# VIPL-Audio-Visual-Speech-Understanding/SBL_For_Multilingual_Lip_Reading

Hardware: AMD Instinct MI355X
Metric: lip-clips/sec fwd+bwd (29x88x88) (higher is better)
Workload: dtype f32 (exact 3-way bf16 split, 6 bf16 MFMA products per fp32 product, fp32 accumulate); 1 GPU; full SBL 6+6 (Conv3d stem + ResNet-18 + encoder + SBL decoder) fwd+loss+bwd (BASELINE config 3); matmul_precision=bf16x6, per_gpu_batch=32, global_batch=32, clip=29x88x88, parallelism=dp1, dropout=True, bn=train, issue=graph, hipgraph=True, decoder_streams=2, conv_weight_pack=cached (re-packed when weights change), decoder_schedule=teacher-forced runs batched, coin_patterns=8

## Files before the change

### include/sbl_hip.h

```cpp
#ifndef SBL_HIP_H
#define SBL_HIP_H
#include <stdint.h>
#ifdef __cplusplus
extern "C" {
#endif

#define SBL_ERR_INVALID (-22)
#define SBL_ABI_VERSION 1

typedef void* sbl_stream_t;

const char* sbl_last_error(void);
int sbl_abi_version(void);

int sbl_profile_begin(uint64_t* stamps, int capacity);
int sbl_profile_end(void);
int sbl_profile_used(void);
int sbl_profile_last_slot(void);
int sbl_profile_last_kernel(void);

int sbl_set_matmul_precision(int terms);
int sbl_get_matmul_precision(void);
int sbl_set_tuning(int knob, int value);

// ... 48 lines not shown
int sbl_bn_bwd_apply(const float* dy, const float* y, const float* x, const float* mean, const float* invstd,
                     const float* gamma, const double* sums, float* dx, float* dres, float* dgamma, float* dbeta,
                     long rows, int C, int relu, int accumulate, sbl_stream_t stream);

int sbl_conv_weight_pack(const float* w_oihw, float* w_ohwi, float* w_dgrad , int Cout,
                         int Cin, int KH, int KW, double* zero , int nzero, sbl_stream_t stream);
int sbl_conv_wgrad_unpack(const float* dw_ohwi, float* dw_oihw, int Cout, int Cin, int KH, int KW, int accumulate,
                          sbl_stream_t stream);
int sbl_conv2d_fwd(const float* x, const float* w_ohwi, float* y, double* stats, int stats_zeroed, int NIMG, int H, int W, int Cin,
                   int Cout, int KH, int KW, int stride, int pad, void* ws, long ws_bytes, sbl_stream_t stream);
int sbl_conv2d_dgrad(const float* dy, const float* w_dgrad, float* dx, int NIMG, int H, int W, int Cin, int Cout,
                     int KH, int KW, int stride, int pad, void* ws, long ws_bytes, sbl_stream_t stream);
int sbl_conv2d_dgrad_bnstats(const float* dy, const float* w_dgrad, float* dx, int NIMG, int H, int W, int Cin, int Cout,
                             int KH, int KW, int stride, int pad, void* ws, long ws_bytes, const float* act,
                             const float* pre, const float* mean, const float* invstd, double* sums,
                             int sums_zeroed ,
                             sbl_stream_t stream);
int sbl_conv2d_dgrad_fused(const float* dy, const float* w_dgrad, float* dx, int NIMG, int H, int W, int Cin, int Cout,
                           int KH, int KW, int stride, int pad, void* ws, long ws_bytes, const float* addend,
                           const float* act, const float* pre, const float* mean, const float* invstd, const float* pre2,
                           const float* mean2, const float* invstd2, double* sums, int sums_zeroed, sbl_stream_t stream);
int sbl_conv1x1s2_dgrad_compact(const float* dy, const float* w_dgrad, float* dx_compact, int NIMG, int H, int W, int Cin,
                                int Cout, void* ws, long ws_bytes, sbl_stream_t stream);
int sbl_conv2d_wgrad(const float* x, const float* dy, float* dw_ohwi, int NIMG, int H, int W, int Cin, int Cout,
                     int KH, int KW, int stride, int pad, int dw_zeroed, sbl_stream_t stream);
int sbl_avgpool_fwd(const float* x, float* y, int NIMG, int HW, int C, sbl_stream_t stream);
int sbl_avgpool_bwd(const float* dy, float* dx, int NIMG, int HW, int C, sbl_stream_t stream);

int sbl_dropout(const float* x, float* y, long n, float p, const uint64_t* seed, uint64_t offset,
                sbl_stream_t stream);
int sbl_seed_bump(uint64_t* seed, sbl_stream_t stream);

int sbl_add_layernorm_fwd(const float* x, const float* res, const float* gamma, const float* beta, float* y,
                          float* mean, float* rstd, int M, int D, float eps, float drop_p, const uint64_t* seed,
                          uint64_t offset, sbl_stream_t stream);
int sbl_add_layernorm2_fusion_fwd(const float* x0, const float* x1, const float* res0, const float* res1, const float* gamma0,
// ... 161 lines not shown
```

### sbl_for_multilingual_lip_reading_amd/csrc/conv.hip

```cpp
#include "mfma_gemm.h"
#include "conv_patch.h"
#include "conv_patch_wgrad.h"

SblRouting g_sbl_route = {2, 30};
extern "C" int sbl_set_tuning(int knob, int value) {
    SBL_REQUIRE(knob == 5 || knob == 9, "sbl_set_tuning: no knob %d; the two that remain are 5 (patch-resident 3x3 / stride-1 forward / input gradient: 2 on, "
                "0 the per-tap gather kernels) and 9 (smallest map in pixels that takes the patch-resident weight gradient, 0 = never)", knob);
    if (knob == 5) {
        SBL_REQUIRE(value == 0 || value == 2, "sbl_set_tuning: knob 5 takes 2 (patch-resident kernels) or 0 (per-tap gather kernels), not %d", value);
        g_sbl_route.conv_patch = value;
    } else {
        SBL_REQUIRE(value >= 0, "sbl_set_tuning: negative value");
        g_sbl_route.conv_patch_wgrad = value;
    }
    return 0;
}

static int check_conv(const char* who, int NIMG, int H, int W, int Cin, int Cout, int KH, int KW, int stride, int pad) {
    SBL_REQUIRE(NIMG > 0 && H > 0 && W > 0, "%s: bad image dims %d %d %d", who, NIMG, H, W);
    SBL_REQUIRE(Cin % 16 == 0 && Cout % 16 == 0 && Cin >= 16 && Cout >= 16, "%s: Cin=%d Cout=%d must be multiples of 16", who, Cin, Cout);
    SBL_REQUIRE((KH == 3 && KW == 3 && pad == 1) || (KH == 1 && KW == 1 && pad == 0), "%s: only 3x3/pad1 and 1x1/pad0 (got %dx%d pad %d)", who, KH, KW, pad);
    SBL_REQUIRE(stride == 1 || stride == 2, "%s: stride %d", who, stride);
    SBL_REQUIRE(sbl_fits_u32((long)NIMG * H * W * (long)(Cin > Cout ? Cin : Cout)), "%s: tensor spans more than 2 GiB (buffer descriptor range)", who);
    SBL_REQUIRE((long)NIMG * H * W < (1L << 24) && Cin < (1 << 16) && Cout < (1 << 16), "%s: more than 2^24 pixels (24-bit index arithmetic in the gathers)", who);
// ... 28 lines not shown
static const RowMap kRowsDirect{0, 0, 0, 0, 0, 0, 0};
static inline RowMap rows_pm(int NIMG, int HW) { return RowMap{2, NIMG, HW, 0, 0, 0, 0}; }

struct DgradFuse {
    const float* addend;
    int add_class00;
    const float* y;
    const float* x;
    const float* mean;
    const float* inv;
    const float* x2;
    const float* mean2;
    const float* inv2;
    double* sums;
    int sums_zeroed;
};

static EpiStore<0, false> epi_plain(float* C, int N, const RowMap& r) {
    return {C, (long)N, nullptr, 0, nullptr, nullptr, 0, r.cmap, r.ca, r.cb, r.cH, r.cW, r.cph, r.cpw};
}
static EpiStore<0, true> epi_stats(float* C, int N, double* stats, const RowMap& r) {
    return {C, (long)N, nullptr, 0, stats, nullptr, 0, r.cmap, r.ca, r.cb, r.cH, r.cW, r.cph, r.cpw};
}
template <bool SUMS>
static EpiStore<0, SUMS, true> epi_fused(float* C, int N, const DgradFuse& f, const float* add, long add_ld, const RowMap& r) {
    const DgradFuse b = SUMS ? f : DgradFuse{};
    return {C, (long)N, nullptr, 0, b.sums, nullptr, 0, r.cmap, r.ca, r.cb, r.cH, r.cW, r.cph, r.cpw,
            b.y, b.x, b.mean, b.inv, b.x2, b.mean2, b.inv2, add, add_ld};
}
template <class F>
static auto with_fwd_epi(float* y, int N, double* stats, const RowMap& r, F&& fn) {
    if (stats) return fn(epi_stats(y, N, stats, r));
    return fn(epi_plain(y, N, r));
}
template <class F>
static auto with_dgrad_epi(float* dx, int N, const DgradFuse& f, F&& fn) {
    if (f.sums) return fn([&](const RowMap& r, const float* add, long add_ld) { return epi_fused<true>(dx, N, f, add, add_ld, r); });
    if (f.addend) return fn([&](const RowMap& r, const float* add, long add_ld) { return epi_fused<false>(dx, N, f, add, add_ld, r); });
    return fn([&](const RowMap& r, const float*, long) { return epi_plain(dx, N, r); });
}

template <class AL, class BL, class EPI, int BM, int BN>
// ... 26 lines not shown
}

extern "C" int sbl_conv2d_fwd(const float* x, const float* w, float* y, double* stats, int stats_zeroed, int NIMG, int H, int W,
                              int Cin, int Cout, int KH, int KW, int stride, int pad, void* ws, long ws_bytes, sbl_stream_t stream) {
    hipStream_t s = (hipStream_t)stream;
    if (int e = check_conv("sbl_conv2d_fwd", NIMG, H, W, Cin, Cout, KH, KW, stride, pad)) return e;
    SBL_REQUIRE(x && w && y && sbl_aligned16(x) && sbl_aligned16(w), "sbl_conv2d_fwd: null/unaligned pointer");
    const int Ho = out_dim(H, KH, stride, pad), Wo = out_dim(W, KW, stride, pad);
    const int M = NIMG * Ho * Wo, N = Cout, K = KH * KW * Cin;
    ConvGeom g{NIMG, Ho, Wo, H, W, Cin, KH, KW, stride, pad, 0, 0, 0, 0, {0, 0, 0, 0}, {0, 0, 0, 0}};
    sbl_geom_finish(g);
    if (stats && !stats_zeroed) SBL_HIP(hipMemsetAsync(stats, 0, sizeof(double) * 2 * Cout, s));
    SBL_REQUIRE(!ws || (sbl_aligned16(ws) && ws_bytes >= (long)sizeof(int) * kConvWsCounters), "sbl_conv2d_fwd: workspace unaligned or < 16 KiB");
    if (KH == 3 && stride == 1) {
        bool done;
        const PatchEpi pe{y, stats, nullptr, nullptr, nullptr, nullptr, nullptr, nullptr, nullptr, nullptr};
        if (stats) done = sbl_launch_conv_patch<false, 1>(x, w, pe, NIMG, H, W, Cin, Cout, SBL_KID_CONV_FWD, s);
        else done = sbl_launch_conv_patch<false, 0>(x, w, pe, NIMG, H, W, Cin, Cout, SBL_KID_CONV_FWD, s);
        if (done) {
            SBL_LAUNCH_CHECK("sbl_conv2d_fwd(patch)");
            return 0;
        }
    }
    if (conv_pm_ok(Ho, Wo, KH, stride)) {
        with_fwd_epi(y, N, stats, rows_pm(NIMG, Ho * Wo), [&](const auto& e) { launch_conv_pm<false>(x, w, g, e, M, N, K, Cin, SBL_KID_CONV_FWD, s); });
        SBL_LAUNCH_CHECK("sbl_conv2d_fwd(pm)");
        return 0;
    }
    const ConvTile tile = conv_tile(N, (long)sbl_cdiv(M, 128) * sbl_cdiv(N, 128), (long)sbl_cdiv(M, 128) * sbl_cdiv(N, 64), true, false);
    with_fwd_epi(y, N, stats, kRowsDirect, [&](const auto& e) { launch_conv_gemm<false>(x, w, g, e, tile, M, N, K, SBL_KID_CONV_FWD, ws, ws_bytes, s); });
    SBL_LAUNCH_CHECK("sbl_conv2d_fwd");
// ... 41 lines not shown
        SplitCtl sc{nullptr, nullptr, nullptr, sbl_next_stamp_slot(SBL_KID_CONV_DGRAD)};
        const int cmap = compact_out ? 0 : 1;
        long t128 = 0, t128x64 = 0;
        for (int i = 0; i < nc; ++i) {
            t128 += (long)sbl_cdiv(cls[i].M, 128) * sbl_cdiv(N, 128);
            t128x64 += (long)sbl_cdiv(cls[i].M, 128) * sbl_cdiv(N, 64);
        }
        const ConvTile tile = conv_tile(N, t128, t128x64, false, f.sums != nullptr);
        int t0[SBL_MAX_CLASSES + 1];
        long tt = 0;
        for (int i = 0; i <= SBL_MAX_CLASSES; ++i) {
            t0[i] = (int)tt;
            if (i < nc) tt += (long)sbl_cdiv(cls[i].M, conv_tile_m(tile)) * sbl_cdiv(N, conv_tile_n(tile));
        }
        SBL_REQUIRE(tt < (1L << 30), "sbl_conv2d_dgrad: too many tiles");
        with_dgrad_epi(dx, N, f, [&](auto make) {
            with_tile(tile, [&](auto bm, auto bn) {
                constexpr int BM = decltype(bm)::value, BN = decltype(bn)::value;
                using AL = ConvGatherKC<BM, true>;
                using BL = DenseKCTaps<BN>;
                using EPI = decltype(make(kRowsDirect, f.addend, 0L));
                ClassSet<AL, BL, EPI> cs;
                cs.nclass = nc;
                cs.tiles_n = sbl_cdiv(N, BN);
                for (int i = 0; i < SBL_MAX_CLASSES; ++i) {
                    const DgradClass& c = cls[i < nc ? i : 0];
                    const float* add = (f.addend && c.ph == 0 && c.pw == 0) ? f.addend : nullptr;
                    cs.al[i] = AL{dy, c.g, c.M};
                    cs.bl[i] = BL{wt, (long)KH * KW * Cout, N, Cout, {c.lin[0], c.lin[1], c.lin[2], c.lin[3]}};
                    cs.epi[i] = make(RowMap{cmap, c.g.OH, c.g.OW, H, W, c.ph, c.pw}, add, (long)N);
                    cs.M[i] = c.M; cs.K[i] = c.K; cs.t0[i] = t0[i];
                }
                cs.t0[SBL_MAX_CLASSES] = t0[SBL_MAX_CLASSES];
                sbl_with_prec([&](auto p) {
                    hipLaunchKernelGGL((sbl_conv_classes_kernel<AL, BL, EPI, BM, BN, decltype(p)::value>), dim3((unsigned)tt), dim3(256), 0, s, cs, sc, N);
                });
            });
        });
        SBL_LAUNCH_CHECK("sbl_conv2d_dgrad(classes)");
        return 0;
    }
    const int M = NIMG * H * W, N = Cin, K = KH * KW * Cout;
    ConvGeom g{NIMG, H, W, Ho, Wo, Cout, KH, KW, stride, pad, 0, 0, 0, 0, {0, 0, 0, 0}, {0, 0, 0, 0}};
    sbl_geom_finish(g);
    SBL_REQUIRE(!ws || (sbl_aligned16(ws) && ws_bytes >= (long)sizeof(int) * kConvWsCounters), "sbl_conv2d_dgrad: workspace unaligned or < 16 KiB");
    if (KH == 3 && stride == 1) {
        bool done;
        const PatchEpi pe{dx, f.sums, f.addend, f.y, f.x, f.mean, f.inv, f.x2, f.mean2, f.inv2};
        if (f.sums) done = sbl_launch_conv_patch<true, 2>(dy, wt, pe, NIMG, H, W, Cout, Cin, SBL_KID_CONV_DGRAD, s);
        else if (f.addend) done = sbl_launch_conv_patch<true, 3>(dy, wt, pe, NIMG, H, W, Cout, Cin, SBL_KID_CONV_DGRAD, s);
        else done = sbl_launch_conv_patch<true, 0>(dy, wt, pe, NIMG, H, W, Cout, Cin, SBL_KID_CONV_DGRAD, s);
        if (done) {
            SBL_LAUNCH_CHECK("sbl_conv2d_dgrad(patch)");
            return 0;
        }
    }
    if (conv_pm_ok(H, W, KH, stride)) {
        with_dgrad_epi(dx, N, f, [&](auto make) {
            launch_conv_pm<true>(dy, wt, g, make(rows_pm(NIMG, H * W), f.addend, 0L), M, N, K, Cout, SBL_KID_CONV_DGRAD, s);
        });
        SBL_LAUNCH_CHECK("sbl_conv2d_dgrad(pm)");
        return 0;
    }
    const ConvTile tile = conv_tile(N, (long)sbl_cdiv(M, 128) * sbl_cdiv(N, 128), (long)sbl_cdiv(M, 128) * sbl_cdiv(N, 64), true, f.sums != nullptr);
    with_dgrad_epi(dx, N, f, [&](auto make) {
        launch_conv_gemm<true>(dy, wt, g, make(kRowsDirect, f.addend, 0L), tile, M, N, K, SBL_KID_CONV_DGRAD, ws, ws_bytes, s);
    });
    SBL_LAUNCH_CHECK("sbl_conv2d_dgrad");
    return 0;
}
static const DgradFuse kNoFuse{nullptr, 0, nullptr, nullptr, nullptr, nullptr, nullptr, nullptr, nullptr, nullptr};
extern "C" int sbl_conv2d_dgrad(const float* dy, const float* wt, float* dx, int NIMG, int H, int W, int Cin, int Cout,
                                int KH, int KW, int stride, int pad, void* ws, long ws_bytes, sbl_stream_t stream) {
    return conv2d_dgrad_impl(dy, wt, dx, NIMG, H, W, Cin, Cout, KH, KW, stride, pad, ws, ws_bytes, stream, kNoFuse, 0);
}
extern "C" int sbl_conv2d_dgrad_bnstats(const float* dy, const float* wt, float* dx, int NIMG, int H, int W, int Cin, int Cout,
                                        int KH, int KW, int stride, int pad, void* ws, long ws_bytes, const float* act,
                                        const float* pre, const float* mean, const float* invstd, double* sums,
                                        int sums_zeroed, sbl_stream_t stream) {
    SBL_REQUIRE(act && pre && mean && invstd && sums, "sbl_conv2d_dgrad_bnstats: null statistics operand");
    return conv2d_dgrad_impl(dy, wt, dx, NIMG, H, W, Cin, Cout, KH, KW, stride, pad, ws, ws_bytes, stream,
                             DgradFuse{nullptr, 0, act, pre, mean, invstd, nullptr, nullptr, nullptr, sums, sums_zeroed}, 0);
}
extern "C" int sbl_conv2d_dgrad_fused(const float* dy, const float* wt, float* dx, int NIMG, int H, int W, int Cin, int Cout,
                                      int KH, int KW, int stride, int pad, void* ws, long ws_bytes, const float* addend,
                                      const float* act, const float* pre, const float* mean, const float* invstd,
                                      const float* pre2, const float* mean2, const float* invstd2, double* sums,
                                      int sums_zeroed, sbl_stream_t stream) {
    return conv2d_dgrad_impl(dy, wt, dx, NIMG, H, W, Cin, Cout, KH, KW, stride, pad, ws, ws_bytes, stream,
                             DgradFuse{addend, addend && stride == 2, act, pre, mean, invstd, pre2, mean2, invstd2, sums, sums_zeroed}, 0);
}
extern "C" int sbl_conv1x1s2_dgrad_compact(const float* dy, const float* wt, float* dx_compact, int NIMG, int H, int W, int Cin,
                                           int Cout, void* ws, long ws_bytes, sbl_stream_t stream) {
    return conv2d_dgrad_impl(dy, wt, dx_compact, NIMG, H, W, Cin, Cout, 1, 1, 2, 0, ws, ws_bytes, stream, kNoFuse, 1);
}

static inline int wgrad_splits(long target, long tiles, int K) {
    int splits = (int)((target + tiles - 1) / tiles);
    if (splits > K / 256) splits = K / 256;
    return splits < 1 ? 1 : splits;
}
extern "C" int sbl_conv2d_wgrad(const float* x, const float* dy, float* dw, int NIMG, int H, int W, int Cin, int Cout,
                                int KH, int KW, int stride, int pad, int dw_zeroed, sbl_stream_t stream) {
    hipStream_t s = (hipStream_t)stream;
    if (int e = check_conv("sbl_conv2d_wgrad", NIMG, H, W, Cin, Cout, KH, KW, stride, pad)) return e;
// ... 127 lines not shown
```

### sbl_for_multilingual_lip_reading_amd/csrc/conv_patch.h

```cpp
#pragma once
#include "mfma_gemm.h"

#define SBL_CP_CK 32
#define SBL_CP_PIXB 64
__device__ __forceinline__ int cp_addr(int row, int chunk) {
    return row * SBL_CP_PIXB + ((chunk ^ ((row >> 2) & 3)) << 4);
}
#define SBL_CP_EROW 68

struct PatchEpi {
    float* out;
    double* stats;
    const float* add_src;
    const float* bs_y;
    const float* bs_x;
    const float* bs_mean;
    const float* bs_inv;
    const float* bs_x2;
    const float* bs_mean2;
    const float* bs_inv2;
};

template <int NT, bool DGRAD, int STATS>
__global__ __launch_bounds__(256) void sbl_conv_patch_kernel(const float* __restrict__ src, const float* __restrict__ wk, PatchEpi epi,
                                                             int NIMG, int H, int W, int C, int Nout, int TR, int tpi, int ntiles, int G,
                                                             unsigned long long* stamp) {
    using Tm = BfTerms<NT>;
    constexpr int NPL = Tm::NPL;
    constexpr int CK = SBL_CP_CK, PIXB = SBL_CP_PIXB, Q4 = CK / 4, WQ = CK / 16;
    constexpr int WPLANE = 64 * PIXB;
    extern __shared__ __attribute__((aligned(16))) unsigned char cp_smem[];
    sbl_stamp_begin(stamp);
    const int tid = threadIdx.x, lane = tid & 63, wave = tid >> 6, half = lane >> 5, l31 = lane & 31;
    const int PW = W + 2, PH = TR + 2;
    const int plane = G * PH * PW * PIXB;
// ... 117 lines not shown
#pragma unroll
            for (int j = 0; j < 2; ++j)
#pragma unroll
                for (int r = 0; r < 16; ++r) {
                    const int pix = (wave * 2 + i) * 32 + (r & 3) + 8 * (r >> 2) + 4 * half;
                    ep[pix * SBL_CP_EROW + j * 32 + l31] = acc[i][j][r];
                }
        __syncthreads();
        for (int pix = tid >> 4; pix < npix; pix += 16) {
            float4 v = *reinterpret_cast<const float4*>(ep + pix * SBL_CP_EROW + ec4);
            const long o = (m0 + pix) * Nout + n0 + ec4;
            if ((STATS == 2 || STATS == 3) && epi.add_src) {
                const float4 a4 = *reinterpret_cast<const float4*>(epi.add_src + o);
                v.x += a4.x; v.y += a4.y; v.z += a4.z; v.w += a4.w;
            }
            *reinterpret_cast<float4*>(epi.out + o) = v;
            if (STATS == 1) {
                st1[0] += v.x; st1[1] += v.y; st1[2] += v.z; st1[3] += v.w;
                st2[0] += v.x * v.x; st2[1] += v.y * v.y; st2[2] += v.z * v.z; st2[3] += v.w * v.w;
            } else if (STATS == 2) {
                const float4 yv = *reinterpret_cast<const float4*>(epi.bs_y + o);
                const float4 xv = *reinterpret_cast<const float4*>(epi.bs_x + o);
                const float g0 = yv.x > 0.f ? v.x : 0.f, g1 = yv.y > 0.f ? v.y : 0.f, g2 = yv.z > 0.f ? v.z : 0.f, g3 = yv.w > 0.f ? v.w : 0.f;
                st1[0] += g0; st1[1] += g1; st1[2] += g2; st1[3] += g3;
                st2[0] += g0 * ((xv.x - emu.x) * eis.x); st2[1] += g1 * ((xv.y - emu.y) * eis.y);
                st2[2] += g2 * ((xv.z - emu.z) * eis.z); st2[3] += g3 * ((xv.w - emu.w) * eis.w);
                if (epi.bs_x2) {
                    const float4 x2 = *reinterpret_cast<const float4*>(epi.bs_x2 + o);
                    st3[0] += g0 * ((x2.x - emu2.x) * eis2.x); st3[1] += g1 * ((x2.y - emu2.y) * eis2.y);
                    st3[2] += g2 * ((x2.z - emu2.z) * eis2.z); st3[3] += g3 * ((x2.w - emu2.w) * eis2.w);
                }
            }
        }
    }
    if (STATS == 1 || STATS == 2) {
        __syncthreads();
        float* red = reinterpret_cast<float*>(cp_smem);
#pragma unroll
        for (int q = 0; q < 4; ++q) {
            red[(0 * 16 + (tid >> 4)) * 64 + ec4 + q] = st1[q];
            red[(1 * 16 + (tid >> 4)) * 64 + ec4 + q] = st2[q];
            red[(2 * 16 + (tid >> 4)) * 64 + ec4 + q] = st3[q];
        }
// ... 70 lines not shown
```

### sbl_for_multilingual_lip_reading_amd/csrc/mfma_gemm.h

```cpp
#pragma once
#include "sbl_common.h"

#include "tile_loaders.h"
#include "tuning.h"

template <int MODE, bool STATS, bool FUSE = false>
struct EpiStore {
    static constexpr bool kStats = STATS;
    static constexpr bool kFuse = FUSE;
    float* C;
    long ldc;
    const float* bias;
    int relu;
    double* stats;
    const float* relu_mask;
    long ldm;
    int cmap, ca, cb, cH, cW, cph, cpw;
    const float* bs_y;
    const float* bs_x;
    const float* bs_mean;
    const float* bs_inv;
    const float* bs_x2;
    const float* bs_mean2;
    const float* bs_inv2;
    const float* add_src;
    long add_ld;
    __device__ __forceinline__ long row_off(int m) const {
// ... 14 lines not shown
        float bmu = 0.f, bis = 0.f, bmu2 = 0.f, bis2 = 0.f;
        if (STATS && bs_y) {
            bmu = bs_mean[n];
            bis = bs_inv[n];
            if (FUSE && bs_x2) {
                bmu2 = bs_mean2[n];
                bis2 = bs_inv2[n];
            }
        }
#pragma unroll
        for (int r = 0; r < 16; ++r) {
            if (FUSE) __builtin_amdgcn_sched_barrier(0);
            const int m = mbase + (r & 3) + 8 * (r >> 2) + 4 * (lane >> 5);
            if (m < M) {
                float v = a[r] + b;
                if (relu) v = fmaxf(v, 0.f);
                if (relu_mask) v = relu_mask[(long)m * ldm + n] > 0.f ? v : 0.f;
                const long o = row_off(m) + n;
                if (FUSE && add_src) v += add_ld ? add_src[(long)m * add_ld + n] : add_src[o];
                float* q = C + o;
                if (MODE == 0) *q = v;
                else if (MODE == 1) *q += v;
                else atomicAdd(q, v);
                if (STATS) {
                    if (bs_y) {
                        const float g = bs_y[o] > 0.f ? v : 0.f;
                        s1 += g;
                        s2 += g * ((bs_x[o] - bmu) * bis);
                        if (FUSE && bs_x2) s3 += g * ((bs_x2[o] - bmu2) * bis2);
                    } else {
                        s1 += v;
                        s2 += v * v;
                    }
                }
            }
// ... 396 lines not shown
```

### sbl_for_multilingual_lip_reading_amd/csrc/norm.hip

```cpp
#include "sbl_common.h"

__global__ __launch_bounds__(256) void bn_apply_fwd_kernel(const float* __restrict__ x, const float* __restrict__ res,
                                                           const float* __restrict__ mean, const float* __restrict__ invstd,
                                                           const float* __restrict__ gamma, const float* __restrict__ beta,
                                                           float* __restrict__ y, long n4, int C4, int relu) {
    for (long i = blockIdx.x * 256L + threadIdx.x; i < n4; i += (long)gridDim.x * 256) {
        const int c = (int)(i % C4) * 4;
        const float4 v = reinterpret_cast<const float4*>(x)[i];
        const float4 mu = *reinterpret_cast<const float4*>(mean + c);
        const float4 is = *reinterpret_cast<const float4*>(invstd + c);
        const float4 ga = *reinterpret_cast<const float4*>(gamma + c);
        const float4 be = *reinterpret_cast<const float4*>(beta + c);
        float4 o;
        o.x = (v.x - mu.x) * is.x * ga.x + be.x;
        o.y = (v.y - mu.y) * is.y * ga.y + be.y;
        o.z = (v.z - mu.z) * is.z * ga.z + be.z;
        o.w = (v.w - mu.w) * is.w * ga.w + be.w;
        if (res) {
            const float4 r = reinterpret_cast<const float4*>(res)[i];
            o.x += r.x; o.y += r.y; o.z += r.z; o.w += r.w;
        }
        if (relu) {
            o.x = fmaxf(o.x, 0.f); o.y = fmaxf(o.y, 0.f); o.z = fmaxf(o.z, 0.f); o.w = fmaxf(o.w, 0.f);
        }
// ... 203 lines not shown
        const float4 is = *reinterpret_cast<const float4*>(invstd + c);
        const float4 ga = *reinterpret_cast<const float4*>(gamma + c);
        const float mg0 = (float)(sums[c] * inv), mg1 = (float)(sums[c + 1] * inv), mg2 = (float)(sums[c + 2] * inv),
                    mg3 = (float)(sums[c + 3] * inv);
        const float mx0 = (float)(sums[C + c] * inv), mx1 = (float)(sums[C + c + 1] * inv),
                    mx2 = (float)(sums[C + c + 2] * inv), mx3 = (float)(sums[C + c + 3] * inv);
        float4 o;
        o.x = ga.x * is.x * (g.x - mg0 - (v.x - mu.x) * is.x * mx0);
        o.y = ga.y * is.y * (g.y - mg1 - (v.y - mu.y) * is.y * mx1);
        o.z = ga.z * is.z * (g.z - mg2 - (v.z - mu.z) * is.z * mx2);
        o.w = ga.w * is.w * (g.w - mg3 - (v.w - mu.w) * is.w * mx3);
        reinterpret_cast<float4*>(dx)[i] = o;
    }
}

static inline int ew_grid(long n) {
    long g = (n + 255) / 256;
    return (int)(g > 8192 ? 8192 : (g < 1 ? 1 : g));
}

extern "C" int sbl_bn_apply_fwd(const float* x, const float* res, const float* mean, const float* invstd,
                                const float* gamma, const float* beta, float* y, long rows, int C, int relu,
                                sbl_stream_t stream) {
    SBL_REQUIRE(x && mean && invstd && gamma && beta && y && rows > 0 && C > 0 && C % 4 == 0, "sbl_bn_apply_fwd: bad args rows=%ld C=%d", rows, C);
    SBL_REQUIRE(sbl_aligned16(x) && sbl_aligned16(y) && (!res || sbl_aligned16(res)), "sbl_bn_apply_fwd: unaligned");
    const long n4 = rows * (C / 4);
    hipLaunchKernelGGL(bn_apply_fwd_kernel, dim3(ew_grid(n4)), dim3(256), 0, (hipStream_t)stream, x, res, mean, invstd,
                       gamma, beta, y, n4, C / 4, relu);
    SBL_LAUNCH_CHECK("sbl_bn_apply_fwd");
    return 0;
// ... 38 lines not shown
        SBL_HIP(hipMemsetAsync(sums, 0, sizeof(double) * 2 * C, s));
    }
    const int rpb = (int)((rows + blocks - 1) / blocks);
    hipLaunchKernelGGL(bn_bwd_reduce_kernel, dim3((int)((rows + rpb - 1) / rpb)), dim3(256), 0, s, dy, y, x, mean, invstd,
                       sums, rows, C, relu, rpb, part, ticket);
    SBL_LAUNCH_CHECK("sbl_bn_bwd_reduce");
    return 0;
}

extern "C" int sbl_bn_bwd_apply(const float* dy, const float* y, const float* x, const float* mean, const float* invstd,
                                const float* gamma, const double* sums, float* dx, float* dres, float* dgamma,
                                float* dbeta, long rows, int C, int relu, int accumulate, sbl_stream_t stream) {
    SBL_REQUIRE(dy && x && mean && invstd && gamma && sums && dx && dgamma && dbeta && rows > 0 && C >= 4 && C % 4 == 0 && (!relu || y),
                "sbl_bn_bwd_apply: bad args");
    const long n4 = rows * (C / 4);
    hipLaunchKernelGGL(bn_bwd_apply_kernel, dim3(ew_grid(n4)), dim3(256), 0, (hipStream_t)stream, dy, y, x, mean, invstd,
                       gamma, sums, dx, dres, dgamma, dbeta, n4, rows, C, relu, accumulate);
    SBL_LAUNCH_CHECK("sbl_bn_bwd_apply");
    return 0;
}

__global__ __launch_bounds__(256) void dropout_kernel(const float* __restrict__ x, float* __restrict__ y, long n,
                                                      uint32_t thresh, float scale, const uint64_t* __restrict__ seed,
                                                      uint64_t offset) {
    const uint64_t sd = *seed;
    for (long i = blockIdx.x * 256L + threadIdx.x; i < n; i += (long)gridDim.x * 256)
        y[i] = sbl_keep(sd, offset, (uint64_t)i, thresh) ? x[i] * scale : 0.f;
}
__global__ void seed_bump_kernel(uint64_t* seed) { *seed = *seed * 6364136223846793005ull + 1442695040888963407ull; }

extern "C" int sbl_dropout(const float* x, float* y, long n, float p, const uint64_t* seed, uint64_t offset,
                           sbl_stream_t stream) {
// ... 413 lines not shown
```

### sbl_for_multilingual_lip_reading_amd/ops.py

```python
import collections as _collections
import copy as _copy
import ctypes as _ct
import functools as _functools
import threading as _threading
import types as _types
import weakref as _weakref

import numpy as _np
import torch
import torch.distributed as _dist

try:
    from . import _lib
except ImportError:
    import _lib

call = _lib.call

_PRECISIONS = {"f32": 0, "bf16x6": 6, "bf16x3": 3, "bf16": 1}


def set_matmul_precision(mode):
    if mode not in _PRECISIONS:
        raise ValueError("matmul precision %r (one of %s)" % (mode, ", ".join(_PRECISIONS)))
# ... 1209 lines not shown
def bn_bwd_apply(dy, y, bn, gamma, beta, sums, with_res):
    conv, mean, invstd = bn
    Cout = conv.size(-1)
    dconv = torch.empty_like(conv)
    dres = torch.empty_like(conv) if with_res else None
    dgamma, dbeta = _gbuf(gamma), _gbuf(beta)
    acc = dgamma is not None and dbeta is not None
    if not acc:
        dgamma = torch.empty(Cout, device=conv.device, dtype=torch.float32)
        dbeta = torch.empty(Cout, device=conv.device, dtype=torch.float32)
    call("sbl_bn_bwd_apply", _p(dy), _p(y), _p(conv), _p(mean), _p(invstd), _p(gamma), _p(sums), _p(dconv), _p(dres),
         _p(dgamma), _p(dbeta), conv.numel() // Cout, Cout, int(y is not None), int(acc), _s())
    return (dconv, dres, None, None) if acc else (dconv, dres, dgamma, dbeta)


def conv_dgrad(dconv, w, w_dg, x, stride, addend=None, bn=None, bn_ds=None):
    Cin = x.size(-1)
    w_dg = _dgrad_weight(w, w_dg)
    dx = torch.empty_like(x)
    n_bn = (bn is not None) + (bn_ds is not None)
    sums, pooled = _zeros_or_empty(x.device, (2 * n_bn * Cin,), torch.float64) if n_bn else (None, False)
    head = (_p(dconv), _p(w_dg), _p(dx), *_conv_geom(x, w, stride), _workspace().data_ptr(), WS_BYTES)
    if addend is None:
        call("sbl_conv2d_dgrad_bnstats", *head, _p(x), *map(_p, bn), _p(sums), int(pooled), _s())
    else:
        call("sbl_conv2d_dgrad_fused", *head, _p(addend), _p(x if n_bn else None), *map(_p, bn or (None,) * 3), *map(_p, bn_ds or (None,) * 3),
             _p(sums), int(pooled), _s())
    return dx, sums


def conv_wgrad(x, dconv, w, stride):
    g = _conv_geom(x, w, stride)
    _, _, _, Cin, Cout, KH, KW, _, _ = g
    dev = x.device

    def launch(dw_ohwi, pooled, target, acc):
        call("sbl_conv2d_wgrad", _p(x), _p(dconv), _p(dw_ohwi), *g, int(pooled), _s())
        call("sbl_conv_wgrad_unpack", _p(dw_ohwi), _p(target), Cout, Cin, KH, KW, acc, _s())

    gw = _gbuf(w)
    if gw is None:
        dw = torch.empty_like(w)
        launch(torch.empty(Cout, KH, KW, Cin, device=dev, dtype=torch.float32), False, dw, 0)
        return dw
    side = side_stream(dev)
    side.wait_stream(torch.cuda.current_stream())
    with torch.cuda.stream(side):
        launch(*_zeros_or_empty(dev, (Cout, KH, KW, Cin), torch.float32), gw, 1)
    x.record_stream(side)
    dconv.record_stream(side)
    _arm_side_join()
    return None


class BlockHandoff:

    __slots__ = ("act", "bn2", "bn_ds", "sums", "dx_ptr")

    def __init__(self):
        self.act = self.bn2 = self.bn_ds = self.sums = self.dx_ptr = None

    def publish(self, y, bn2, bn_ds):
        self.act, self.bn2, self.bn_ds = y.data_ptr(), bn2, bn_ds

    def describes(self, x):
        return self.bn2 is not None and self.act == x.data_ptr()

    def deposit(self, sums, dx):
        self.sums, self.dx_ptr = sums, dx.data_ptr()

    def take(self, dy):
        if self.sums is None or self.dx_ptr != dy.data_ptr():
            return None
        sums = self.sums
        self.__init__()
        return sums


class BlockFn(torch.autograd.Function):

    @staticmethod
    def forward(ctx, x, prev, pub, c1, c2, ds, training, *params):
        _need_cuda(x, *params)
        x = x.contiguous()
        need_dx = ctx.needs_input_grad[0]
        conv1, out, mean1, invstd1, w_dg1 = conv_bn_fwd(x, c1, None, True, training, need_dx)
        res, bn_ds, saved_ds = x, None, ()
        if ds is not None:
            conv_ds, res, mean_ds, invstd_ds, w_dg_ds = conv_bn_fwd(x, ds, None, False, training, need_dx)
            bn_ds, saved_ds = (conv_ds, mean_ds, invstd_ds), (conv_ds, mean_ds, invstd_ds, w_dg_ds)
        need_dout = pub is not None and (need_dx or any(ctx.needs_input_grad[7:10]))
# ... 3 lines not shown
        if pub is not None:
            pub.publish(y, (conv2, mean2, invstd2), bn_ds)
        return y

    @staticmethod
    @_bw
    def backward(ctx, dy):
        if not ctx.training:
            raise _lib.SblHipError("ConvBN backward is implemented for training-mode BatchNorm only")
        x, conv1, out, mean1, invstd1, w_dg1, conv2, y, mean2, invstd2, w_dg2, *params = ctx.saved_tensors
        w1, gamma1, beta1, w2, gamma2, beta2, *ds = params
        stride1, stride_ds = ctx.strides
        need_dx = ctx.needs_input_grad[0]
        bn1, bn2 = (conv1, mean1, invstd1), (conv2, mean2, invstd2)
        dy = dy.contiguous()
        sums2 = ctx.pub.take(dy) if ctx.pub is not None else None
        sums_ds = None
        if sums2 is None:
            sums2 = bn_bwd_reduce(dy, y, bn2)
        elif ds:
            sums2, sums_ds = sums2[:sums2.numel() // 2], sums2[sums2.numel() // 2:]
        dconv2, dres, dgamma2, dbeta2 = bn_bwd_apply(dy, y, bn2, gamma2, beta2, sums2, True)
        dout, sums1 = conv_dgrad(dconv2, w2, w_dg2, out, 1, bn=bn1)
        dw2 = conv_wgrad(out, dconv2, w2, 1)
        grads_ds, addend = (), dres
        if ds:
            w_ds, gamma_ds, beta_ds, conv_ds, mean_ds, invstd_ds, w_dg_ds = ds
            bn_ds = (conv_ds, mean_ds, invstd_ds)
            if sums_ds is None:
                sums_ds = bn_bwd_reduce(dres, None, bn_ds)
            dconv_ds, _, dgamma_ds, dbeta_ds = bn_bwd_apply(dres, None, bn_ds, gamma_ds, beta_ds, sums_ds, False)
            if need_dx:
                NIMG, H, W, Cin = x.shape
                addend = torch.empty(NIMG, (H + 1) // 2, (W + 1) // 2, Cin, device=x.device, dtype=torch.float32)
                call("sbl_conv1x1s2_dgrad_compact", _p(dconv_ds), _p(_dgrad_weight(w_ds, w_dg_ds)), _p(addend), NIMG, H, W, Cin,
                     w_ds.size(0), _workspace().data_ptr(), WS_BYTES, _s())
            grads_ds = (conv_wgrad(x, dconv_ds, w_ds, stride_ds), dgamma_ds, dbeta_ds)
        dconv1, _, dgamma1, dbeta1 = bn_bwd_apply(dout, out, bn1, gamma1, beta1, sums1, False)
        dx = None
        if need_dx:
            prev = ctx.prev if ctx.prev is not None and ctx.prev.describes(x) else None
            if prev is None:
                dx, _ = conv_dgrad(dconv1, w1, w_dg1, x, stride1, addend)
            else:
                dx, sums_prev = conv_dgrad(dconv1, w1, w_dg1, x, stride1, addend, prev.bn2, prev.bn_ds)
                prev.deposit(sums_prev, dx)
        dw1 = conv_wgrad(x, dconv1, w1, stride1)
        return (dx, None, None, None, None, None, None, dw1, dgamma1, dbeta1, dw2, dgamma2, dbeta2, *grads_ds)


def basic_block(x, c1, c2, ds, training):
    pub = BlockHandoff() if training and torch.is_grad_enabled() else None
    y = BlockFn.apply(x, getattr(x, "_sbl_handoff", None), pub, c1, c2, ds, training, *c1[:3], *c2[:3], *(ds[:3] if ds is not None else ()))
    if pub is not None:
        y._sbl_handoff = pub
    return y


class AvgPoolFn(torch.autograd.Function):

    @staticmethod
# ... 429 lines not shown
```

Before: 1031 clips/s.

## Store ReLU-masked gradients from dgrad epilogue and add vectorized BN-backward apply kernel

The fused dgrad epilogue (patch-resident and class-tiled paths) can now write the ReLU-masked gradient instead of the raw one, controlled by a new flags bit. Downstream BN-backward apply calls in the ResNet blocks then skip the activation read and masking, and the residual gradient is reused directly instead of being rewritten. A separate BN-backward apply kernel hoists per-channel constants out of the loop when C/4 divides the block size. The change adds a hard error for a 128x128 tile with the stats+fuse epilogue, which could abort if that tile is ever picked.

Result: no change. 1034 clips/s, median of 4 (+0.3%).

```diff
diff --git a/include/sbl_hip.h b/include/sbl_hip.h
--- a/include/sbl_hip.h
+++ b/include/sbl_hip.h
@@ -86,12 +86,12 @@
 int sbl_conv2d_dgrad_bnstats(const float* dy, const float* w_dgrad, float* dx, int NIMG, int H, int W, int Cin, int Cout,
                              int KH, int KW, int stride, int pad, void* ws, long ws_bytes, const float* act,
                              const float* pre, const float* mean, const float* invstd, double* sums,
-                             int sums_zeroed ,
+                             int flags,
                              sbl_stream_t stream);
 int sbl_conv2d_dgrad_fused(const float* dy, const float* w_dgrad, float* dx, int NIMG, int H, int W, int Cin, int Cout,
                            int KH, int KW, int stride, int pad, void* ws, long ws_bytes, const float* addend,
                            const float* act, const float* pre, const float* mean, const float* invstd, const float* pre2,
-                           const float* mean2, const float* invstd2, double* sums, int sums_zeroed, sbl_stream_t stream);
+                           const float* mean2, const float* invstd2, double* sums, int flags, sbl_stream_t stream);
 int sbl_conv1x1s2_dgrad_compact(const float* dy, const float* w_dgrad, float* dx_compact, int NIMG, int H, int W, int Cin,
                                 int Cout, void* ws, long ws_bytes, sbl_stream_t stream);
 int sbl_conv2d_wgrad(const float* x, const float* dy, float* dw_ohwi, int NIMG, int H, int W, int Cin, int Cout,
diff --git a/sbl_for_multilingual_lip_reading_amd/csrc/conv.hip b/sbl_for_multilingual_lip_reading_amd/csrc/conv.hip
--- a/sbl_for_multilingual_lip_reading_amd/csrc/conv.hip
+++ b/sbl_for_multilingual_lip_reading_amd/csrc/conv.hip
@@ -66,6 +66,7 @@
     const float* inv2;
     double* sums;
     int sums_zeroed;
+    int store_g;
 };
 
 static EpiStore<0, false> epi_plain(float* C, int N, const RowMap& r) {
@@ -77,7 +78,7 @@
 template <bool SUMS>
 static EpiStore<0, SUMS, true> epi_fused(float* C, int N, const DgradFuse& f, const float* add, long add_ld, const RowMap& r) {
     const DgradFuse b = SUMS ? f : DgradFuse{};
-    return {C, (long)N, nullptr, 0, b.sums, nullptr, 0, r.cmap, r.ca, r.cb, r.cH, r.cW, r.cph, r.cpw,
+    return {C, (long)N, nullptr, b.store_g ? EpiStore<0, SUMS, true>::kStoreG : 0, b.sums, nullptr, 0, r.cmap, r.ca, r.cb, r.cH, r.cW, r.cph, r.cpw,
             b.y, b.x, b.mean, b.inv, b.x2, b.mean2, b.inv2, add, add_ld};
 }
 template <class F>
@@ -134,7 +135,7 @@
     SBL_REQUIRE(!ws || (sbl_aligned16(ws) && ws_bytes >= (long)sizeof(int) * kConvWsCounters), "sbl_conv2d_fwd: workspace unaligned or < 16 KiB");
     if (KH == 3 && stride == 1) {
         bool done;
-        const PatchEpi pe{y, stats, nullptr, nullptr, nullptr, nullptr, nullptr, nullptr, nullptr, nullptr};
+        const PatchEpi pe{y, stats, nullptr, nullptr, nullptr, nullptr, nullptr, nullptr, nullptr, nullptr, 0};
         if (stats) done = sbl_launch_conv_patch<false, 1>(x, w, pe, NIMG, H, W, Cin, Cout, SBL_KID_CONV_FWD, s);
         else done = sbl_launch_conv_patch<false, 0>(x, w, pe, NIMG, H, W, Cin, Cout, SBL_KID_CONV_FWD, s);
         if (done) {
@@ -206,12 +207,15 @@
             if (i < nc) tt += (long)sbl_cdiv(cls[i].M, conv_tile_m(tile)) * sbl_cdiv(N, conv_tile_n(tile));
         }
         SBL_REQUIRE(tt < (1L << 30), "sbl_conv2d_dgrad: too many tiles");
+        bool no_kernel = false;
         with_dgrad_epi(dx, N, f, [&](auto make) {
             with_tile(tile, [&](auto bm, auto bn) {
                 constexpr int BM = decltype(bm)::value, BN = decltype(bn)::value;
                 using AL = ConvGatherKC<BM, true>;
                 using BL = DenseKCTaps<BN>;
                 using EPI = decltype(make(kRowsDirect, f.addend, 0L));
+                if constexpr (BN == 128 && EPI::kStats && EPI::kFuse) no_kernel = true;
+                else {
                 ClassSet<AL, BL, EPI> cs;
                 cs.nclass = nc;
                 cs.tiles_n = sbl_cdiv(N, BN);
@@ -227,8 +231,10 @@
                 sbl_with_prec([&](auto p) {
                     hipLaunchKernelGGL((sbl_conv_classes_kernel<AL, BL, EPI, BM, BN, decltype(p)::value>), dim3((unsigned)tt), dim3(256), 0, s, cs, sc, N);
                 });
+                }
             });
         });
+        SBL_REQUIRE(!no_kernel, "sbl_conv2d_dgrad(classes): no 128x128 kernel with the sums epilogue");
         SBL_LAUNCH_CHECK("sbl_conv2d_dgrad(classes)");
         return 0;
     }
@@ -238,7 +244,7 @@
     SBL_REQUIRE(!ws || (sbl_aligned16(ws) && ws_bytes >= (long)sizeof(int) * kConvWsCounters), "sbl_conv2d_dgrad: workspace unaligned or < 16 KiB");
     if (KH == 3 && stride == 1) {
         bool done;
-        const PatchEpi pe{dx, f.sums, f.addend, f.y, f.x, f.mean, f.inv, f.x2, f.mean2, f.inv2};
+        const PatchEpi pe{dx, f.sums, f.addend, f.y, f.x, f.mean, f.inv, f.x2, f.mean2, f.inv2, f.sums ? f.store_g : 0};
         if (f.sums) done = sbl_launch_conv_patch<true, 2>(dy, wt, pe, NIMG, H, W, Cout, Cin, SBL_KID_CONV_DGRAD, s);
         else if (f.addend) done = sbl_launch_conv_patch<true, 3>(dy, wt, pe, NIMG, H, W, Cout, Cin, SBL_KID_CONV_DGRAD, s);
         else done = sbl_launch_conv_patch<true, 0>(dy, wt, pe, NIMG, H, W, Cout, Cin, SBL_KID_CONV_DGRAD, s);
@@ -261,7 +267,8 @@
     SBL_LAUNCH_CHECK("sbl_conv2d_dgrad");
     return 0;
 }
-static const DgradFuse kNoFuse{nullptr, 0, nullptr, nullptr, nullptr, nullptr, nullptr, nullptr, nullptr, nullptr};
+static const DgradFuse kNoFuse{nullptr, 0, nullptr, nullptr, nullptr, nullptr, nullptr, nullptr, nullptr, nullptr, 0, 0};
+static inline bool dgrad_flags_ok(int flags, const double* sums) { return (flags & ~3) == 0 && (!(flags & 2) || sums); }
 extern "C" int sbl_conv2d_dgrad(const float* dy, const float* wt, float* dx, int NIMG, int H, int W, int Cin, int Cout,
                                 int KH, int KW, int stride, int pad, void* ws, long ws_bytes, sbl_stream_t stream) {
     return conv2d_dgrad_impl(dy, wt, dx, NIMG, H, W, Cin, Cout, KH, KW, stride, pad, ws, ws_bytes, stream, kNoFuse, 0);
@@ -269,18 +276,20 @@
 extern "C" int sbl_conv2d_dgrad_bnstats(const float* dy, const float* wt, float* dx, int NIMG, int H, int W, int Cin, int Cout,
                                         int KH, int KW, int stride, int pad, void* ws, long ws_bytes, const float* act,
                                         const float* pre, const float* mean, const float* invstd, double* sums,
-                                        int sums_zeroed, sbl_stream_t stream) {
+                                        int flags, sbl_stream_t stream) {
     SBL_REQUIRE(act && pre && mean && invstd && sums, "sbl_conv2d_dgrad_bnstats: null statistics operand");
+    SBL_REQUIRE(dgrad_flags_ok(flags, sums), "sbl_conv2d_dgrad_bnstats: bad flags %d", flags);
     return conv2d_dgrad_impl(dy, wt, dx, NIMG, H, W, Cin, Cout, KH, KW, stride, pad, ws, ws_bytes, stream,
-                             DgradFuse{nullptr, 0, act, pre, mean, invstd, nullptr, nullptr, nullptr, sums, sums_zeroed}, 0);
+                             DgradFuse{nullptr, 0, act, pre, mean, invstd, nullptr, nullptr, nullptr, sums, flags & 1, (flags >> 1) & 1}, 0);
 }
 extern "C" int sbl_conv2d_dgrad_fused(const float* dy, const float* wt, float* dx, int NIMG, int H, int W, int Cin, int Cout,
                                       int KH, int KW, int stride, int pad, void* ws, long ws_bytes, const float* addend,
                                       const float* act, const float* pre, const float* mean, const float* invstd,
                                       const float* pre2, const float* mean2, const float* invstd2, double* sums,
-                                      int sums_zeroed, sbl_stream_t stream) {
+                                      int flags, sbl_stream_t stream) {
+    SBL_REQUIRE(dgrad_flags_ok(flags, sums), "sbl_conv2d_dgrad_fused: bad flags %d (bit 1 needs the BatchNorm operands)", flags);
     return conv2d_dgrad_impl(dy, wt, dx, NIMG, H, W, Cin, Cout, KH, KW, stride, pad, ws, ws_bytes, stream,
-                             DgradFuse{addend, addend && stride == 2, act, pre, mean, invstd, pre2, mean2, invstd2, sums, sums_zeroed}, 0);
+                             DgradFuse{addend, addend && stride == 2, act, pre, mean, invstd, pre2, mean2, invstd2, sums, flags & 1, (flags >> 1) & 1}, 0);
 }
 extern "C" int sbl_conv1x1s2_dgrad_compact(const float* dy, const float* wt, float* dx_compact, int NIMG, int H, int W, int Cin,
                                            int Cout, void* ws, long ws_bytes, sbl_stream_t stream) {
diff --git a/sbl_for_multilingual_lip_reading_amd/csrc/conv_patch.h b/sbl_for_multilingual_lip_reading_amd/csrc/conv_patch.h
--- a/sbl_for_multilingual_lip_reading_amd/csrc/conv_patch.h
+++ b/sbl_for_multilingual_lip_reading_amd/csrc/conv_patch.h
@@ -19,6 +19,7 @@
     const float* bs_x2;
     const float* bs_mean2;
     const float* bs_inv2;
+    int store_g;
 };
 
 template <int NT, bool DGRAD, int STATS>
@@ -166,19 +167,21 @@
                 const float4 a4 = *reinterpret_cast<const float4*>(epi.add_src + o);
                 v.x += a4.x; v.y += a4.y; v.z += a4.z; v.w += a4.w;
             }
-            *reinterpret_cast<float4*>(epi.out + o) = v;
+            if (STATS != 2 || !epi.store_g) *reinterpret_cast<float4*>(epi.out + o) = v;
             if (STATS == 1) {
                 st1[0] += v.x; st1[1] += v.y; st1[2] += v.z; st1[3] += v.w;
                 st2[0] += v.x * v.x; st2[1] += v.y * v.y; st2[2] += v.z * v.z; st2[3] += v.w * v.w;
             } else if (STATS == 2) {
                 const float4 yv = *reinterpret_cast<const float4*>(epi.bs_y + o);
                 const float4 xv = *reinterpret_cast<const float4*>(epi.bs_x + o);
+                float4 x2 = make_float4(0.f, 0.f, 0.f, 0.f);
+                if (epi.bs_x2) x2 = *reinterpret_cast<const float4*>(epi.bs_x2 + o);
                 const float g0 = yv.x > 0.f ? v.x : 0.f, g1 = yv.y > 0.f ? v.y : 0.f, g2 = yv.z > 0.f ? v.z : 0.f, g3 = yv.w > 0.f ? v.w : 0.f;
+                if (epi.store_g) *reinterpret_cast<float4*>(epi.out + o) = make_float4(g0, g1, g2, g3);
                 st1[0] += g0; st1[1] += g1; st1[2] += g2; st1[3] += g3;
                 st2[0] += g0 * ((xv.x - emu.x) * eis.x); st2[1] += g1 * ((xv.y - emu.y) * eis.y);
                 st2[2] += g2 * ((xv.z - emu.z) * eis.z); st2[3] += g3 * ((xv.w - emu.w) * eis.w);
                 if (epi.bs_x2) {
-                    const float4 x2 = *reinterpret_cast<const float4*>(epi.bs_x2 + o);
                     st3[0] += g0 * ((x2.x - emu2.x) * eis2.x); st3[1] += g1 * ((x2.y - emu2.y) * eis2.y);
                     st3[2] += g2 * ((x2.z - emu2.z) * eis2.z); st3[3] += g3 * ((x2.w - emu2.w) * eis2.w);
                 }
diff --git a/sbl_for_multilingual_lip_reading_amd/csrc/mfma_gemm.h b/sbl_for_multilingual_lip_reading_amd/csrc/mfma_gemm.h
--- a/sbl_for_multilingual_lip_reading_amd/csrc/mfma_gemm.h
+++ b/sbl_for_multilingual_lip_reading_amd/csrc/mfma_gemm.h
@@ -11,6 +11,7 @@
     float* C;
     long ldc;
     const float* bias;
+    static constexpr int kStoreG = 2;
     int relu;
     double* stats;
     const float* relu_mask;
@@ -55,11 +56,20 @@
             const int m = mbase + (r & 3) + 8 * (r >> 2) + 4 * (lane >> 5);
             if (m < M) {
                 float v = a[r] + b;
-                if (relu) v = fmaxf(v, 0.f);
+                if (FUSE ? (relu & 1) : relu) v = fmaxf(v, 0.f);
                 if (relu_mask) v = relu_mask[(long)m * ldm + n] > 0.f ? v : 0.f;
                 const long o = row_off(m) + n;
                 if (FUSE && add_src) v += add_ld ? add_src[(long)m * add_ld + n] : add_src[o];
                 float* q = C + o;
+                if (FUSE && STATS && MODE == 0 && bs_y && (relu & kStoreG)) {
+                    const float yv = bs_y[o], xv = bs_x[o], xv2 = bs_x2 ? bs_x2[o] : 0.f;
+                    const float g = yv > 0.f ? v : 0.f;
+                    *q = g;
+                    s1 += g;
+                    s2 += g * ((xv - bmu) * bis);
+                    if (bs_x2) s3 += g * ((xv2 - bmu2) * bis2);
+                    continue;
+                }
                 if (MODE == 0) *q = v;
                 else if (MODE == 1) *q += v;
                 else atomicAdd(q, v);
diff --git a/sbl_for_multilingual_lip_reading_amd/csrc/norm.hip b/sbl_for_multilingual_lip_reading_amd/csrc/norm.hip
--- a/sbl_for_multilingual_lip_reading_amd/csrc/norm.hip
+++ b/sbl_for_multilingual_lip_reading_amd/csrc/norm.hip
@@ -241,6 +241,49 @@
     }
 }
 
+__global__ __launch_bounds__(256) void bn_bwd_apply_quad_kernel(const float* __restrict__ dy, const float* __restrict__ y,
+                                                                const float* __restrict__ x, const float* __restrict__ mean,
+                                                                const float* __restrict__ invstd, const float* __restrict__ gamma,
+                                                                const double* __restrict__ sums, float* __restrict__ dx,
+                                                                float* __restrict__ dres, float* __restrict__ dgamma,
+                                                                float* __restrict__ dbeta, long n4, long rows, int C, int relu,
+                                                                int accumulate) {
+    const int C4 = C / 4;
+    const double inv = 1.0 / (double)rows;
+    if (blockIdx.x == 0)
+        for (int c = threadIdx.x; c < C; c += 256) {
+            dbeta[c] = (accumulate ? dbeta[c] : 0.f) + (float)sums[c];
+            dgamma[c] = (accumulate ? dgamma[c] : 0.f) + (float)sums[C + c];
+        }
+    const long i0 = blockIdx.x * 256L + threadIdx.x;
+    const int c = (int)(i0 % C4) * 4;
+    const float4 mu = *reinterpret_cast<const float4*>(mean + c);
+    const float4 is = *reinterpret_cast<const float4*>(invstd + c);
+    const float4 ga = *reinterpret_cast<const float4*>(gamma + c);
+    const float mg0 = (float)(sums[c] * inv), mg1 = (float)(sums[c + 1] * inv), mg2 = (float)(sums[c + 2] * inv),
+                mg3 = (float)(sums[c + 3] * inv);
+    const float mx0 = (float)(sums[C + c] * inv), mx1 = (float)(sums[C + c + 1] * inv),
+                mx2 = (float)(sums[C + c + 2] * inv), mx3 = (float)(sums[C + c + 3] * inv);
+    for (long i = i0; i < n4; i += (long)gridDim.x * 256) {
+        float4 g = reinterpret_cast<const float4*>(dy)[i];
+        if (relu) {
+            const float4 yy = reinterpret_cast<const float4*>(y)[i];
+            if (!(yy.x > 0.f)) g.x = 0.f;
+            if (!(yy.y > 0.f)) g.y = 0.f;
+            if (!(yy.z > 0.f)) g.z = 0.f;
+            if (!(yy.w > 0.f)) g.w = 0.f;
+        }
+        if (dres) reinterpret_cast<float4*>(dres)[i] = g;
+        const float4 v = reinterpret_cast<const float4*>(x)[i];
+        float4 o;
+        o.x = ga.x * is.x * (g.x - mg0 - (v.x - mu.x) * is.x * mx0);
+        o.y = ga.y * is.y * (g.y - mg1 - (v.y - mu.y) * is.y * mx1);
+        o.z = ga.z * is.z * (g.z - mg2 - (v.z - mu.z) * is.z * mx2);
+        o.w = ga.w * is.w * (g.w - mg3 - (v.w - mu.w) * is.w * mx3);
+        reinterpret_cast<float4*>(dx)[i] = o;
+    }
+}
+
 static inline int ew_grid(long n) {
     long g = (n + 255) / 256;
     return (int)(g > 8192 ? 8192 : (g < 1 ? 1 : g));
@@ -309,8 +352,9 @@
     SBL_REQUIRE(dy && x && mean && invstd && gamma && sums && dx && dgamma && dbeta && rows > 0 && C >= 4 && C % 4 == 0 && (!relu || y),
                 "sbl_bn_bwd_apply: bad args");
     const long n4 = rows * (C / 4);
-    hipLaunchKernelGGL(bn_bwd_apply_kernel, dim3(ew_grid(n4)), dim3(256), 0, (hipStream_t)stream, dy, y, x, mean, invstd,
-                       gamma, sums, dx, dres, dgamma, dbeta, n4, rows, C, relu, accumulate);
+    const bool quad = (C / 4) <= 256 && 256 % (C / 4) == 0;
+    hipLaunchKernelGGL(quad ? bn_bwd_apply_quad_kernel : bn_bwd_apply_kernel, dim3(ew_grid(n4)), dim3(256), 0, (hipStream_t)stream,
+                       dy, y, x, mean, invstd, gamma, sums, dx, dres, dgamma, dbeta, n4, rows, C, relu, accumulate);
     SBL_LAUNCH_CHECK("sbl_bn_bwd_apply");
     return 0;
 }
diff --git a/sbl_for_multilingual_lip_reading_amd/ops.py b/sbl_for_multilingual_lip_reading_amd/ops.py
--- a/sbl_for_multilingual_lip_reading_amd/ops.py
+++ b/sbl_for_multilingual_lip_reading_amd/ops.py
@@ -1247,18 +1247,22 @@
     return (dconv, dres, None, None) if acc else (dconv, dres, dgamma, dbeta)
 
 
-def conv_dgrad(dconv, w, w_dg, x, stride, addend=None, bn=None, bn_ds=None):
+MASKED_TRUNK_GRADS = True
+
+
+def conv_dgrad(dconv, w, w_dg, x, stride, addend=None, bn=None, bn_ds=None, masked=False):
     Cin = x.size(-1)
     w_dg = _dgrad_weight(w, w_dg)
     dx = torch.empty_like(x)
     n_bn = (bn is not None) + (bn_ds is not None)
     sums, pooled = _zeros_or_empty(x.device, (2 * n_bn * Cin,), torch.float64) if n_bn else (None, False)
     head = (_p(dconv), _p(w_dg), _p(dx), *_conv_geom(x, w, stride), _workspace().data_ptr(), WS_BYTES)
+    flags = int(pooled) | (2 if masked and bn is not None else 0)
     if addend is None:
-        call("sbl_conv2d_dgrad_bnstats", *head, _p(x), *map(_p, bn), _p(sums), int(pooled), _s())
+        call("sbl_conv2d_dgrad_bnstats", *head, _p(x), *map(_p, bn), _p(sums), flags, _s())
     else:
         call("sbl_conv2d_dgrad_fused", *head, _p(addend), _p(x if n_bn else None), *map(_p, bn or (None,) * 3), *map(_p, bn_ds or (None,) * 3),
-             _p(sums), int(pooled), _s())
+             _p(sums), flags, _s())
     return dx, sums
 
 
@@ -1288,10 +1292,11 @@
 
 class BlockHandoff:
 
-    __slots__ = ("act", "bn2", "bn_ds", "sums", "dx_ptr")
+    __slots__ = ("act", "bn2", "bn_ds", "sums", "dx_ptr", "masked")
 
     def __init__(self):
         self.act = self.bn2 = self.bn_ds = self.sums = self.dx_ptr = None
+        self.masked = False
 
     def publish(self, y, bn2, bn_ds):
         self.act, self.bn2, self.bn_ds = y.data_ptr(), bn2, bn_ds
@@ -1299,15 +1304,15 @@
     def describes(self, x):
         return self.bn2 is not None and self.act == x.data_ptr()
 
-    def deposit(self, sums, dx):
-        self.sums, self.dx_ptr = sums, dx.data_ptr()
+    def deposit(self, sums, dx, masked=False):
+        self.sums, self.dx_ptr, self.masked = sums, dx.data_ptr(), masked
 
     def take(self, dy):
         if self.sums is None or self.dx_ptr != dy.data_ptr():
-            return None
-        sums = self.sums
+            return None, False
+        got = (self.sums, self.masked)
         self.__init__()
-        return sums
+        return got
 
 
 class BlockFn(torch.autograd.Function):
@@ -1341,14 +1346,19 @@
         need_dx = ctx.needs_input_grad[0]
         bn1, bn2 = (conv1, mean1, invstd1), (conv2, mean2, invstd2)
         dy = dy.contiguous()
-        sums2 = ctx.pub.take(dy) if ctx.pub is not None else None
+        sums2, dy_masked = ctx.pub.take(dy) if ctx.pub is not None else (None, False)
         sums_ds = None
         if sums2 is None:
             sums2 = bn_bwd_reduce(dy, y, bn2)
         elif ds:
             sums2, sums_ds = sums2[:sums2.numel() // 2], sums2[sums2.numel() // 2:]
-        dconv2, dres, dgamma2, dbeta2 = bn_bwd_apply(dy, y, bn2, gamma2, beta2, sums2, True)
-        dout, sums1 = conv_dgrad(dconv2, w2, w_dg2, out, 1, bn=bn1)
+        if dy_masked:
+            dconv2, _, dgamma2, dbeta2 = bn_bwd_apply(dy, None, bn2, gamma2, beta2, sums2, False)
+            dres = dy
+        else:
+            dconv2, dres, dgamma2, dbeta2 = bn_bwd_apply(dy, y, bn2, gamma2, beta2, sums2, True)
+        masked = bool(MASKED_TRUNK_GRADS)
+        dout, sums1 = conv_dgrad(dconv2, w2, w_dg2, out, 1, bn=bn1, masked=masked)
         dw2 = conv_wgrad(out, dconv2, w2, 1)
         grads_ds, addend = (), dres
         if ds:
@@ -1363,15 +1373,15 @@
                 call("sbl_conv1x1s2_dgrad_compact", _p(dconv_ds), _p(_dgrad_weight(w_ds, w_dg_ds)), _p(addend), NIMG, H, W, Cin,
                      w_ds.size(0), _workspace().data_ptr(), WS_BYTES, _s())
             grads_ds = (conv_wgrad(x, dconv_ds, w_ds, stride_ds), dgamma_ds, dbeta_ds)
-        dconv1, _, dgamma1, dbeta1 = bn_bwd_apply(dout, out, bn1, gamma1, beta1, sums1, False)
+        dconv1, _, dgamma1, dbeta1 = bn_bwd_apply(dout, None if masked else out, bn1, gamma1, beta1, sums1, False)
         dx = None
         if need_dx:
             prev = ctx.prev if ctx.prev is not None and ctx.prev.describes(x) else None
             if prev is None:
                 dx, _ = conv_dgrad(dconv1, w1, w_dg1, x, stride1, addend)
             else:
-                dx, sums_prev = conv_dgrad(dconv1, w1, w_dg1, x, stride1, addend, prev.bn2, prev.bn_ds)
-                prev.deposit(sums_prev, dx)
+                dx, sums_prev = conv_dgrad(dconv1, w1, w_dg1, x, stride1, addend, prev.bn2, prev.bn_ds, masked=masked)
+                prev.deposit(sums_prev, dx, masked)
         dw1 = conv_wgrad(x, dconv1, w1, stride1)
         return (dx, None, None, None, None, None, None, dw1, dgamma1, dbeta1, dw2, dgamma2, dbeta2, *grads_ds)
 
```
